# facebookresearch/DRTK

Hardware: AMD Instinct MI355X
Metric: Mpixels/sec fwd+bwd, 100k-tri @ 2048x2048, 1/2/4/8 GPU; HBM BW % (higher is better)
Workload: dtype f32; 1 GPU; 8 views/GPU x 1 GPU, 100k-tri UV-sphere head mesh (F=100352, V=50400), 2048x2048, C=16 attribute channels, transform+rasterize+render+interpolate+mask+edge_grad_estimator+loss fwd+bwd; views_per_gpu=8, triangles=100352, vertices=50400, height=2048, width=2048, channels=16, grad_reset=set_to_none, parallelism=single GPU

## Files before the change

drtk_amd/csrc/edge_grad.hip:

```cpp
#include <cstdlib>

#include "common.hpp"
#include "segscatter.hpp"

namespace drtk_amd {
namespace {

template <typename T>
struct Vec4;
template <>
struct Vec4<float> {
  using type = float4;
};
template <>
struct Vec4<double> {
  using type = double4;
};

template <typename T>
using Quad = T __attribute__((ext_vector_type(4), aligned(sizeof(T))));

template <typename T, int VEC>
struct Row {
  T v[VEC];
  T next;
};

template <typename T, int VEC>
__device__ __forceinline__ Row<T, VEC> load_row(
    const T* __restrict__ plane, int64_t row_off, int x, int W, bool x_ok, int lane) {
  Row<T, VEC> r;
  if (x_ok) {
    if constexpr (VEC == 4) {
      if (x + 4 <= W) {
        const Quad<T> q = *reinterpret_cast<const Quad<T>*>(plane + row_off + x);
        r.v[0] = q.x, r.v[1] = q.y, r.v[2] = q.z, r.v[3] = q.w;
      } else {
#pragma unroll
        for (int j = 0; j < 4; ++j) r.v[j] = x + j < W ? plane[row_off + x + j] : T(0);
      }
    } else {
      r.v[0] = plane[row_off + x];
    }
  } else {
#pragma unroll
    for (int j = 0; j < VEC; ++j) r.v[j] = T(0);
  }
  r.next = __shfl_down(r.v[0], 1);
  return r;
}

#ifndef DRTK_EDGE_SLOTS
#define DRTK_EDGE_SLOTS 64
#endif
#ifndef DRTK_ONEPASS_CAP
#define DRTK_ONEPASS_CAP 512
#endif
#ifndef DRTK_ONEPASS_WAVES
#define DRTK_ONEPASS_WAVES 6
#endif
constexpr int kOnepassCap = DRTK_ONEPASS_CAP;

template <typename T>
struct PairArgs {
  const T* v_pix;
  const int32_t* vi;
  const T* bary_img;
  T* grad_v_pix;
  int64_t V, vi_sN;
  T M;
};

__device__ __forceinline__ int prefix4(int cnt, unsigned long long lt, int& total) {
  const unsigned long long b0 = __ballot(cnt & 1), b1 = __ballot(cnt & 2), b2 = __ballot(cnt & 4);
  total = __popcll(b0) + 2 * __popcll(b1) + 4 * __popcll(b2);
  return __popcll(b0 & lt) + 2 * __popcll(b1 & lt) + 4 * __popcll(b2 & lt);
}

template <typename T, int AXIS, int SLOTS>
__device__ __forceinline__ void scatter_pair_round(
    bool act, int px, int y, T term, const int32_t* __restrict__ idx_n, const T* __restrict__ v_n,
    const int32_t* __restrict__ vi_n, const T* __restrict__ bary_n, int64_t HW, int W, T M, int32_t* keys,
    TableAcc* vals, T* __restrict__ grad_n);

template <typename T, int VEC, int R, int WAVES, bool SCATTER = false>
__global__ __launch_bounds__(WAVES * kWave, SCATTER ? DRTK_ONEPASS_WAVES : 1) void edge_dots_kernel(
    const T* __restrict__ img, const T* __restrict__ grad_output, const int32_t* __restrict__ index_img, int C,
    int H, int W, int strips_x, T* __restrict__ gdx, T* __restrict__ gdy, int strip, T* __restrict__ zero_out,
    int64_t zero_count, PairArgs<T> pairs) {
  static_assert(!SCATTER || (VEC == 4 && 8 * R <= 32 && sizeof(T) == 4), "the pair phase works on four-pixel lanes of float; its flags are one register");
  if (zero_out) {
    const int64_t step = int64_t(gridDim.x) * gridDim.y * blockDim.x;
    for (int64_t i = (int64_t(blockIdx.y) * gridDim.x + blockIdx.x) * blockDim.x + threadIdx.x; i < zero_count; i += step) zero_out[i] = T(0);
  }
  const int64_t HW = int64_t(H) * W;
  const int n = blockIdx.y;
  const int tile = tile_index(strip);
  const int by = tile / strips_x, sx = tile - by * strips_x;
  const int lane = threadIdx.x & (kWave - 1);
  const int y0 = (by * WAVES + threadIdx.x / kWave) * R;
  if (y0 >= H) return;
  const int x = (sx * (kWave - 1) + lane) * VEC;
  const T* img_n = img + int64_t(n) * C * HW;
  const T* go_n = grad_output + int64_t(n) * C * HW;

  bool any_fg = false;
  uint32_t flags = 0;
  {
    const int32_t* idx_n = index_img + int64_t(n) * HW;
    int32_t above[4] = {-1, -1, -1, -1};
#pragma unroll
    for (int r = 0; r <= R; ++r) {
      const int y = y0 + r;
      if (y < H) {
        bool fg = false;
        int32_t first = -1, last = -1;
        int32_t cur[4] = {-1, -1, -1, -1};
        if (x < W) {
          if constexpr (VEC == 4) {
            Quad<int32_t> q;
            if (x + 4 <= W) {
              q = *reinterpret_cast<const Quad<int32_t>*>(idx_n + int64_t(y) * W + x);
            } else {
              const int32_t* rp = idx_n + int64_t(y) * W + x;
              q.x = rp[0], q.y = x + 1 < W ? rp[1] : -1, q.z = x + 2 < W ? rp[2] : -1, q.w = -1;
            }
            fg = (q.x & q.y & q.z & q.w) != -1;
            first = q.x, last = q.w;
            cur[0] = q.x, cur[1] = q.y, cur[2] = q.z, cur[3] = q.w;
          } else {
            first = last = idx_n[int64_t(y) * W + x];
            fg = first != -1;
          }
        }
        int32_t left = __shfl_up(last, 1), right = __shfl_down(first, 1);
        if (lane == 0) left = (x >= 1 && x < W) ? idx_n[int64_t(y) * W + x - 1] : -1;
        if (lane == kWave - 1) right = (x + VEC < W) ? idx_n[int64_t(y) * W + x + VEC] : -1;
        any_fg = any_fg || fg || left != -1 || right != -1;
        if constexpr (SCATTER) {
#pragma unroll
          for (int j = 0; j < 4; ++j) {
            const bool in_x = lane != kWave - 1 && x + j < W - 1;
            if (r > 0 && in_x && above[j] != cur[j]) flags |= 1u << (4 * R + 4 * (r - 1) + j);
            const int32_t nr = j < 3 ? cur[(j + 1) & 3] : right;
            if (r < R && in_x && y < H - 1 && cur[j] != nr) flags |= 1u << (4 * r + j);
            above[j] = cur[j];
          }
        }
      }
    }
  }
  bool load_any = any_fg;
  if constexpr (SCATTER) {
    if (__ballot(flags != 0) == 0) return;
    uint32_t h3 = 0;
#pragma unroll
    for (int r = 0; r < R; ++r) h3 |= flags & (8u << (4 * r));
    const int left_h3 = __shfl_up(static_cast<int>(h3), 1);
    load_any = flags != 0 || (lane > 0 && left_h3 != 0);
  } else {
    if (__ballot(any_fg) == 0) return;
  }
  const bool x_ok = x < W && load_any;

  T ax[R][VEC], ay[R][VEC];
#pragma unroll
  for (int r = 0; r < R; ++r)
#pragma unroll
    for (int j = 0; j < VEC; ++j) ax[r][j] = ay[r][j] = T(0);

  for (int c = 0; c < C; ++c) {
    const T* ip = img_n + int64_t(c) * HW;
    const T* gp = go_n + int64_t(c) * HW;
    Row<T, VEC> ri[R + 1], rg[R + 1];
#pragma unroll
    for (int r = 0; r <= R; ++r) {
      const bool y_ok = (y0 + r) < H;
      ri[r] = load_row<T, VEC>(ip, int64_t(y0 + r) * W, x, W, x_ok && y_ok, lane);
      rg[r] = load_row<T, VEC>(gp, int64_t(y0 + r) * W, x, W, x_ok && y_ok, lane);
    }
#pragma unroll
    for (int r = 0; r < R; ++r) {
#pragma unroll
      for (int j = 0; j < VEC; ++j) {
        const T inext = (j + 1 < VEC) ? ri[r].v[(j + 1) % VEC] : ri[r].next;
        const T gnext = (j + 1 < VEC) ? rg[r].v[(j + 1) % VEC] : rg[r].next;
        ax[r][j] += (inext - ri[r].v[j]) * (T(0.5) * (gnext + rg[r].v[j]));
        ay[r][j] += (ri[r + 1].v[j] - ri[r].v[j]) * (T(0.5) * (rg[r + 1].v[j] + rg[r].v[j]));
      }
    }
  }
  if constexpr (SCATTER) {
    constexpr int kSlots = DRTK_EDGE_SLOTS;
    constexpr int kCap = kOnepassCap;
    __shared__ uint2 s_list[WAVES][kCap];
    __shared__ int32_t t_keys[WAVES][kSlots];
    __shared__ TableAcc t_vals[WAVES][kSlots * 4];
    const int wave = threadIdx.x / kWave;
    const int32_t* idx_n = index_img + int64_t(n) * HW;
    const T* v_n = pairs.v_pix + int64_t(n) * pairs.V * 3;
    const int32_t* vi_n = pairs.vi + int64_t(n) * pairs.vi_sN;
    const T* bary_n = pairs.bary_img + int64_t(n) * 3 * HW;
    T* grad_n = pairs.grad_v_pix + int64_t(n) * pairs.V * 3;
    const int strip_x0 = sx * (kWave - 1) * VEC;

    table_init<kSlots>(t_keys[wave]);
    for (int i = lane; i < kSlots * 4; i += kWave) t_vals[wave][i] = 0;

    const unsigned long long lt = (1ull << lane) - 1ull;
    int grand = 0;
#pragma unroll
    for (int g = 0; g < 2 * R; ++g) {
      int t;
      prefix4(__popc((flags >> (4 * g)) & 15u), lt, t);
      grand += t;
    }
    if (grand <= kCap) {
      int n_h = 0, n_all = 0;
#pragma unroll
      for (int axis = 0; axis < 2; ++axis) {
#pragma unroll
        for (int r = 0; r < R; ++r) {
          const uint32_t f = (flags >> (4 * R * axis + 4 * r)) & 15u;
          int t;
          int pos = n_all + prefix4(__popc(f), lt, t);
          n_all += t;
#pragma unroll
          for (int j = 0; j < 4; ++j) {
            if (f & (1u << j)) s_list[wave][pos++] = make_uint2((r << 8) | (lane * 4 + j), __builtin_bit_cast(uint32_t, axis == 0 ? ax[r][j] : ay[r][j]));
          }
        }
        if (axis == 0) n_h = n_all;
      }
      wave_lds_sync();

      for (int axis = 0; axis < 2; ++axis) {
        const int l_begin = axis == 0 ? 0 : n_h, l_end = axis == 0 ? n_h : n_all;
        for (int t0 = l_begin; t0 < l_end; t0 += kWave) {
          const int t = t0 + lane;
          const bool act = t < l_end;
          int px = 0, y = 0;
          T term = T(0);
          if (act) {
            const uint2 entry = s_list[wave][t];
            y = y0 + static_cast<int>(entry.x >> 8);
            px = strip_x0 + static_cast<int>(entry.x & 255u);
            term = __builtin_bit_cast(float, entry.y);
          }
          if (axis == 0) {
            scatter_pair_round<T, 0, kSlots>(act, px, y, term, idx_n, v_n, vi_n, bary_n, HW, W, pairs.M, t_keys[wave], t_vals[wave], grad_n);
          } else {
            scatter_pair_round<T, 1, kSlots>(act, px, y, term, idx_n, v_n, vi_n, bary_n, HW, W, pairs.M, t_keys[wave], t_vals[wave], grad_n);
          }
        }
      }
    } else {
      static_assert(2 * kCap >= kWave * 8 * R, "the list's storage must hold a strip's terms");
      uint32_t* s_terms = reinterpret_cast<uint32_t*>(s_list[wave]);
#pragma unroll
      for (int q = 0; q < 4 * R; ++q) {
        s_terms[q * kWave + lane] = __builtin_bit_cast(uint32_t, ax[q / 4][q % 4]);
        s_terms[(4 * R + q) * kWave + lane] = __builtin_bit_cast(uint32_t, ay[q / 4][q % 4]);
      }
      wave_lds_sync();
      for (int axis = 0; axis < 2; ++axis) {
#pragma unroll 1
        for (int k = 0; k < 4 * R; ++k) {
          const bool act = (flags >> (4 * R * axis + k)) & 1u;
          if (__ballot(act) == 0) continue;
          const T term = __builtin_bit_cast(float, s_terms[(4 * R * axis + k) * kWave + lane]);
          if (axis == 0) {
            scatter_pair_round<T, 0, kSlots>(act, x + (k & 3), y0 + (k >> 2), term, idx_n, v_n, vi_n, bary_n, HW, W, pairs.M, t_keys[wave], t_vals[wave], grad_n);
          } else {
            scatter_pair_round<T, 1, kSlots>(act, x + (k & 3), y0 + (k >> 2), term, idx_n, v_n, vi_n, bary_n, HW, W, pairs.M, t_keys[wave], t_vals[wave], grad_n);
          }
        }
      }
    }
    wave_lds_sync();
    table_flush<T, TableAcc, kSlots>(t_keys[wave], t_vals[wave], 4, 3, grad_n, 3, 0);
    return;
  }
  if (!x_ok || lane == kWave - 1) return;
  T* ox = gdx + int64_t(n) * HW;
  T* oy = gdy + int64_t(n) * HW;
#pragma unroll
  for (int r = 0; r < R; ++r) {
    const int y = y0 + r;
    if (y >= H) break;
    const int64_t o = int64_t(y) * W + x;
    if constexpr (VEC == 4) {
      if (x + 4 <= W) {
        *reinterpret_cast<Quad<T>*>(ox + o) = Quad<T>{ax[r][0], ax[r][1], ax[r][2], ax[r][3]};
        *reinterpret_cast<Quad<T>*>(oy + o) = Quad<T>{ay[r][0], ay[r][1], ay[r][2], ay[r][3]};
      } else {
#pragma unroll
        for (int j = 0; j < 4; ++j)
          if (x + j < W) ox[o + j] = ax[r][j], oy[o + j] = ay[r][j];
      }
    } else {
      ox[o] = ax[r][0];
      oy[o] = ay[r][0];
    }
  }
}

template <typename T>
struct TriInfo {
  T p0x, p0y, p1x, p1y;
  T v01x, v01y, v02x, v02y, v12x, v12y;
  T den;
  T nx, ny, nz;
  int32_t i0, i1, i2;
};

template <typename T>
__device__ __forceinline__ void load_tri(
    const T* __restrict__ v_n, const int32_t* __restrict__ vi_n, int32_t idx, TriInfo<T>& t) {
  t.i0 = t.i1 = t.i2 = 0;
  if (idx >= 0) {
    const int32_t* f = vi_n + int64_t(idx) * 3;
    t.i0 = f[0], t.i1 = f[1], t.i2 = f[2];
  }
  t.p0x = v_n[3 * (int64_t)t.i0 + 0];
  t.p0y = v_n[3 * (int64_t)t.i0 + 1];
  t.p1x = v_n[3 * (int64_t)t.i1 + 0];
  t.p1y = v_n[3 * (int64_t)t.i1 + 1];
  const T p2x = v_n[3 * (int64_t)t.i2 + 0], p2y = v_n[3 * (int64_t)t.i2 + 1];
  t.v01x = t.p1x - t.p0x;
  t.v01y = t.p1y - t.p0y;
  t.v02x = p2x - t.p0x;
  t.v02y = p2y - t.p0y;
  t.v12x = p2x - t.p1x;
  t.v12y = p2y - t.p1y;
  t.den = t.v01x * t.v02y - t.v01y * t.v02x;
}

template <typename T>
__device__ __forceinline__ bool pix_in_tri(const TriInfo<T>& t, int x, int y) {
  if (t.den != T(0)) {
    const T px = static_cast<T>(x), py = static_cast<T>(y);
    const T vp0x = px - t.p0x, vp0y = py - t.p0y;
    const T vp1x = px - t.p1x, vp1y = py - t.p1y;
    T b0 = vp1y * t.v12x - vp1x * t.v12y;
    T b1 = vp0x * t.v02y - vp0y * t.v02x;
    T b2 = vp0y * t.v01x - vp0x * t.v01y;
    const T s = t.den > T(0) ? T(1) : (t.den < T(0) ? T(-1) : T(0));
    b0 *= s;
    b1 *= s;
    b2 *= s;
    const bool inside = (b0 >= T(0)) && (b1 >= T(0)) && (b2 >= T(0));
    const bool on0 = b0 == T(0), on1 = b1 == T(0), on2 = b2 == T(0);
    const bool pos = t.den > T(0);
    const bool tl0 = pos ? (t.v12y < T(0) || (t.v12y == T(0) && t.v12x > T(0)))
                         : (t.v12y > T(0) || (t.v12y == T(0) && t.v12x < T(0)));
    const bool tl1 = pos ? (t.v02y > T(0) || (t.v02y == T(0) && t.v02x < T(0)))
                         : (t.v02y < T(0) || (t.v02y == T(0) && t.v02x > T(0)));
    const bool tl2 = pos ? (t.v01y < T(0) || (t.v01y == T(0) && t.v01x > T(0)))
                         : (t.v01y > T(0) || (t.v01y == T(0) && t.v01x < T(0)));
    return inside && !((on0 && !tl0) || (on1 && !tl1) || (on2 && !tl2));
  }
  return false;
}

__device__ __forceinline__ float sqrt_t(float x) {
  return __builtin_sqrtf(x);
}
__device__ __forceinline__ double sqrt_t(double x) {
  return __builtin_sqrt(x);
}

template <typename T>
__device__ __forceinline__ void tri_normal(const T* __restrict__ v_n, TriInfo<T>& t) {
  const T* p0 = v_n + 3 * (int64_t)t.i0;
  const T* p1 = v_n + 3 * (int64_t)t.i1;
  const T* p2 = v_n + 3 * (int64_t)t.i2;
  const T ax = p0[0] - p2[0], ay = p0[1] - p2[1], az = p0[2] - p2[2];
  const T bx = p1[0] - p0[0], by = p1[1] - p0[1], bz = p1[2] - p0[2];
  const T cx = ay * bz - az * by;
  const T cy = az * bx - ax * bz;
  const T cz = ax * by - ay * bx;
  const T inv = T(1.0) / sqrt_t(cx * cx + cy * cy + cz * cz);
  t.nx = cx * inv;
  t.ny = cy * inv;
  t.nz = cz * inv;
}

template <typename T>
__device__ __forceinline__ void get_dp_dr(T nvx, T nvy, T nfx, T nfy, T M, T& ox, T& oy) {
  const T inv_v = T(1.0) / sqrt_t(nvx * nvx + nvy * nvy);
  const T nv_x = nvx * inv_v, nv_y = nvy * inv_v;
  const T inv_f = T(1.0) / sqrt_t(nfx * nfx + nfy * nfy);
  const T nf_x = nfx * inv_f, nf_y = nfy * inv_f;
  const T bx = -nf_y, by = nf_x;
  const T d = bx * nv_x + by * nv_y;
  T q;
  if (M > T(0)) {
    const T abs_d = d < T(0) ? -d : d;
    const T abs_bx = bx < T(0) ? -bx : bx;
    const T lim = abs_bx / M;
    const T m = abs_d < lim ? lim : abs_d;
    const T safe_d = (d >= T(0) ? T(1) : T(-1)) * epsclamp(m);
    q = bx / safe_d;
  } else {
    q = bx / epsclamp(d);
  }
  ox = q * nv_x;
  oy = q * nv_y;
}

template <typename T, int AXIS>
__device__ __forceinline__ void eval_pair(
    const T* __restrict__ v_n, TriInfo<T>& tA, TriInfo<T>& tB, int32_t idxA, int32_t idxB, int xa,
    int ya, T grad_dot, T M, T& gA, T& zA, T& gB, T& zB) {
  gA = zA = gB = zB = T(0);
  const bool a_valid = idxA >= 0, b_valid = idxB >= 0;
  const bool both = a_valid && b_valid;
  const int xb = xa + (AXIS == 0 ? 1 : 0), yb = ya + (AXIS == 1 ? 1 : 0);
  const bool a_in_b = both && pix_in_tri(tB, xa, ya);
  const bool b_in_a = both && pix_in_tri(tA, xb, yb);
  const bool a_over_b = a_in_b && !b_in_a;
  const bool b_over_a = b_in_a && !a_in_b;
  const bool inter = a_in_b && b_in_a;
  const bool adjacent = both && !a_in_b && !b_in_a;
  if (!inter) {
    gA = (!a_valid || b_over_a || adjacent) ? T(0) : grad_dot;
    gB = (!b_valid || a_over_b || adjacent) ? T(0) : grad_dot;
  } else {
    tri_normal(v_n, tA);
    tri_normal(v_n, tB);
    const T a_in = AXIS == 0 ? tA.nx : tA.ny;
    const T b_in = AXIS == 0 ? tB.nx : tB.ny;
    T dx, dz;
    get_dp_dr<T>(a_in, tA.nz, b_in, tB.nz, M, dx, dz);
    gA = grad_dot * dx;
    zA = grad_dot * dz;
    get_dp_dr<T>(b_in, tB.nz, a_in, tA.nz, M, dx, dz);
    gB = grad_dot * dx;
    zB = grad_dot * dz;
  }
}

template <typename T>
__device__ __forceinline__ void edge_pixel(
    const T* __restrict__ v_n, const int32_t* __restrict__ vi_n, const T* __restrict__ gdx_n,
    const T* __restrict__ gdy_n, int64_t pix, int x, int y, int W, int32_t ic, int32_t ir, int32_t id,
    int32_t il, int32_t iu, T M, T& ox, T& oy, T& oz, int32_t* centre_vids = nullptr) {
  T cx = T(0), cy = T(0), cz = T(0);
  T rx = T(0), rz = T(0);
  T dy = T(0), dz = T(0);
  TriInfo<T> tc;
  load_tri<T>(v_n, vi_n, ic, tc);
  if (centre_vids) {
    centre_vids[0] = tc.i0, centre_vids[1] = tc.i1, centre_vids[2] = tc.i2;
  }
  T gA, zA, gB, zB;
  if (ic != ir) {
    TriInfo<T> tn;
    load_tri<T>(v_n, vi_n, ir, tn);
    eval_pair<T, 0>(v_n, tc, tn, ic, ir, x, y, gdx_n[pix], M, gA, zA, gB, zB);
    cx += gA;
    cz += zA;
  }
  if (ic != id) {
    TriInfo<T> tn;
    load_tri<T>(v_n, vi_n, id, tn);
    eval_pair<T, 1>(v_n, tc, tn, ic, id, x, y, gdy_n[pix], M, gA, zA, gB, zB);
    cy += gA;
    cz += zA;
  }
  if (il != ic) {
    TriInfo<T> tn;
    load_tri<T>(v_n, vi_n, il, tn);
    eval_pair<T, 0>(v_n, tn, tc, il, ic, x - 1, y, gdx_n[pix - 1], M, gA, zA, gB, zB);
    rx += gB;
    rz += zB;
  }
  if (iu != ic) {
    TriInfo<T> tn;
    load_tri<T>(v_n, vi_n, iu, tn);
    eval_pair<T, 1>(v_n, tn, tc, iu, ic, x, y - 1, gdy_n[pix - W], M, gA, zA, gB, zB);
    dy += gB;
    dz += zB;
  }
  ox = (T(0) + (-rx)) + (-cx);
  oy = (T(0) + (-dy)) + (-cy);
  oz = ((T(0) + (-dz)) + (-rz)) + (-cz);
}

template <typename T>
__global__ __launch_bounds__(kBlock) void edge_gather_kernel(
    const T* __restrict__ v_pix, const int32_t* __restrict__ vi,
    const int32_t* __restrict__ index_img, const T* __restrict__ gdx, const T* __restrict__ gdy,
    int64_t V, int64_t vi_sN, int H, int W, T M, T* __restrict__ out) {
  const int64_t HW = int64_t(H) * W;
  const int n = blockIdx.y;
  const int64_t pix = int64_t(blockIdx.x) * kBlock + threadIdx.x;
  if (pix >= HW) return;
  const int y = static_cast<int>(pix / W);
  const int x = static_cast<int>(pix - int64_t(y) * W);
  const int32_t* idx_n = index_img + int64_t(n) * HW;

  const bool own = (x < W - 1) && (y < H - 1);
  const bool left = (x >= 1) && (y < H - 1);
  const bool up = (y >= 1) && (x < W - 1);
  const int32_t ic = idx_n[pix];
  const int32_t ir = own ? idx_n[pix + 1] : ic;
  const int32_t id = own ? idx_n[pix + W] : ic;
  const int32_t il = left ? idx_n[pix - 1] : ic;
  const int32_t iu = up ? idx_n[pix - W] : ic;
  T ox = T(0), oy = T(0), oz = T(0);
  if (ic != ir || ic != id || ic != il || ic != iu) {
    edge_pixel<T>(
        v_pix + int64_t(n) * V * 3, vi + int64_t(n) * vi_sN, gdx + int64_t(n) * HW, gdy + int64_t(n) * HW, pix,
        x, y, W, ic, ir, id, il, iu, M, ox, oy, oz);
  }
  T* o = out + int64_t(n) * 3 * HW + pix;
  o[0] = ox;
  o[HW] = oy;
  o[2 * HW] = oz;
}

template <typename T>
__global__ __launch_bounds__(kBlock) void edge_gather4_kernel(
    const T* __restrict__ v_pix, const int32_t* __restrict__ vi,
    const int32_t* __restrict__ index_img, const T* __restrict__ gdx, const T* __restrict__ gdy,
    int64_t V, int64_t vi_sN, int H, int W, T M, T* __restrict__ out, int strip) {
  using V4 = typename Vec4<T>::type;
  constexpr int kWaves = kBlock / kWave;
  constexpr int kPix = kWave * 4;
  __shared__ __attribute__((aligned(16))) T s_out[kWaves][3][kPix];
  __shared__ uint16_t s_list[kWaves][kPix];
  __shared__ int32_t s_nb[kWaves][4][kPix];

  const int64_t HW = int64_t(H) * W;
  const int n = blockIdx.y;
  const int wave = threadIdx.x / kWave, lane = threadIdx.x & (kWave - 1);
  const int64_t wave_pix0 = (int64_t(tile_index(strip)) * kWaves + wave) * kPix;
  if (wave_pix0 >= HW) return;
  const int64_t pix0 = wave_pix0 + lane * 4;
  const bool in_range = pix0 < HW;
  const int32_t* idx_n = index_img + int64_t(n) * HW;
  const int y = in_range ? static_cast<int>(pix0 / W) : 0;
  const int x0 = in_range ? static_cast<int>(pix0 - int64_t(y) * W) : 0;

  int32_t c[4] = {-1, -1, -1, -1}, u[4], d[4];
  if (in_range) {
    const int4 q = *reinterpret_cast<const int4*>(idx_n + pix0);
    c[0] = q.x, c[1] = q.y, c[2] = q.z, c[3] = q.w;
  }
#pragma unroll
  for (int j = 0; j < 4; ++j) u[j] = d[j] = c[j];
  if (in_range && y >= 1) {
    const int4 q = *reinterpret_cast<const int4*>(idx_n + pix0 - W);
    u[0] = q.x, u[1] = q.y, u[2] = q.z, u[3] = q.w;
  }
  if (in_range && y < H - 1) {
    const int4 q = *reinterpret_cast<const int4*>(idx_n + pix0 + W);
    d[0] = q.x, d[1] = q.y, d[2] = q.z, d[3] = q.w;
  }
  int32_t lprev = __shfl_up(c[3], 1), rnext = __shfl_down(c[0], 1);
  if (in_range && lane == 0 && x0 >= 1) lprev = idx_n[pix0 - 1];
  if (in_range && lane == kWave - 1 && x0 + 4 < W) rnext = idx_n[pix0 + 4];

  bool e[4];
  int32_t nr[4], nd[4], nl[4], nu[4];
#pragma unroll
  for (int j = 0; j < 4; ++j) {
    const int x = x0 + j;
    const bool own = in_range && (x < W - 1) && (y < H - 1);
    const bool left = in_range && (x >= 1) && (y < H - 1);
    const bool up = in_range && (y >= 1) && (x < W - 1);
    nr[j] = own ? (j < 3 ? c[(j + 1) & 3] : rnext) : c[j];
    nd[j] = own ? d[j] : c[j];
    nl[j] = left ? (j > 0 ? c[(j + 3) & 3] : lprev) : c[j];
    nu[j] = up ? u[j] : c[j];
    e[j] = c[j] != nr[j] || c[j] != nd[j] || c[j] != nl[j] || c[j] != nu[j];
  }

  const V4 zero4 = V4{T(0), T(0), T(0), T(0)};
#pragma unroll
  for (int k = 0; k < 3; ++k) *reinterpret_cast<V4*>(&s_out[wave][k][lane * 4]) = zero4;
  *reinterpret_cast<int4*>(&s_nb[wave][0][lane * 4]) = make_int4(nr[0], nr[1], nr[2], nr[3]);
  *reinterpret_cast<int4*>(&s_nb[wave][1][lane * 4]) = make_int4(nd[0], nd[1], nd[2], nd[3]);
  *reinterpret_cast<int4*>(&s_nb[wave][2][lane * 4]) = make_int4(nl[0], nl[1], nl[2], nl[3]);
  *reinterpret_cast<int4*>(&s_nb[wave][3][lane * 4]) = make_int4(nu[0], nu[1], nu[2], nu[3]);
  const unsigned long long lt = (1ull << lane) - 1ull;
  int total = 0;
#pragma unroll
  for (int j = 0; j < 4; ++j) {
    const unsigned long long m = __ballot(e[j]);
    if (e[j]) s_list[wave][total + __popcll(m & lt)] = static_cast<uint16_t>(lane * 4 + j);
    total += __popcll(m);
  }
  wave_lds_sync();

  const T* v_n = v_pix + int64_t(n) * V * 3;
  const int32_t* vi_n = vi + int64_t(n) * vi_sN;
  const T* gdx_n = gdx + int64_t(n) * HW;
  const T* gdy_n = gdy + int64_t(n) * HW;
  for (int t0 = 0; t0 < total; t0 += kWave) {
    const int t = t0 + lane;
    if (t < total) {
      const int local = s_list[wave][t];
      const int64_t pix = wave_pix0 + local;
      const int py = static_cast<int>(pix / W);
      const int px = static_cast<int>(pix - int64_t(py) * W);
      const int32_t ic = idx_n[pix];
      T ox, oy, oz;
      edge_pixel<T>(
          v_n, vi_n, gdx_n, gdy_n, pix, px, py, W, ic, s_nb[wave][0][local], s_nb[wave][1][local],
          s_nb[wave][2][local], s_nb[wave][3][local], M, ox, oy, oz);
      s_out[wave][0][local] = ox;
      s_out[wave][1][local] = oy;
      s_out[wave][2][local] = oz;
    }
  }
  wave_lds_sync();
  if (in_range) {
    T* o = out + int64_t(n) * 3 * HW + pix0;
#pragma unroll
    for (int k = 0; k < 3; ++k) *reinterpret_cast<V4*>(o + int64_t(k) * HW) = *reinterpret_cast<const V4*>(&s_out[wave][k][lane * 4]);
  }
}

template <typename T, int AXIS, int SLOTS>
__device__ __forceinline__ void scatter_pair_round(
    bool act, int px, int y, T term, const int32_t* __restrict__ idx_n, const T* __restrict__ v_n,
    const int32_t* __restrict__ vi_n, const T* __restrict__ bary_n, int64_t HW, int W, T M, int32_t* keys,
    TableAcc* vals, T* __restrict__ grad_n) {
  int32_t ia = -1, ib = -1;
  T ga = T(0), za = T(0), gb = T(0), zb = T(0);
  T Ba[3] = {T(0), T(0), T(0)}, Bb[3] = {T(0), T(0), T(0)};
  int32_t va[3] = {0, 0, 0}, vb[3] = {0, 0, 0};
  if (act) {
    const int64_t pa = int64_t(y) * W + px;
    const int64_t pb = AXIS == 0 ? pa + 1 : pa + W;
    ia = idx_n[pa];
    ib = idx_n[pb];
    TriInfo<T> ta, tb;
    load_tri<T>(v_n, vi_n, ia, ta);
    load_tri<T>(v_n, vi_n, ib, tb);
    T gA, zA, gB, zB;
    eval_pair<T, AXIS>(v_n, ta, tb, ia, ib, px, y, term, M, gA, zA, gB, zB);
    ga = -gA, za = -zA, gb = -gB, zb = -zB;
    va[0] = ta.i0, va[1] = ta.i1, va[2] = ta.i2;
    vb[0] = tb.i0, vb[1] = tb.i1, vb[2] = tb.i2;
    if (ia >= 0) Ba[0] = bary_n[pa], Ba[1] = bary_n[HW + pa], Ba[2] = bary_n[2 * HW + pa];
    if (ib >= 0) Bb[0] = bary_n[pb], Bb[1] = bary_n[HW + pb], Bb[2] = bary_n[2 * HW + pb];
  }
  const bool a_on = ia >= 0 && (ga != T(0) || za != T(0));
  const bool b_on = ib >= 0 && (gb != T(0) || zb != T(0));
  T g[12];
#pragma unroll
  for (int k = 0; k < 3; ++k) {
    g[2 * k + 0] = a_on ? ga * Ba[k] : T(0);
    g[2 * k + 1] = a_on ? za * Ba[k] : T(0);
    g[6 + 2 * k + 0] = b_on ? gb * Bb[k] : T(0);
    g[6 + 2 * k + 1] = b_on ? zb * Bb[k] : T(0);
  }
  const int32_t key_a = a_on ? ia : -1, key_b = b_on ? ib : -1;
  int dist;
  bool tail;
  const int32_t left_a = __shfl_up(key_a, 1), left_b = __shfl_up(key_b, 1);
  run_rows16_heads(key_a != left_a || key_b != left_b, dist, tail);
  if (__ballot(a_on || b_on) != 0) {
    run_sums_rows16<T, 12>(g, dist);
    constexpr int c_off = AXIS == 0 ? 0 : 1, c_step = AXIS == 0 ? 2 : 1;
    if (tail && a_on) table_add<T, 3, 2, SLOTS>(keys, vals, 4, va, g, grad_n, 3, c_off, c_step);
    if (tail && b_on) table_add<T, 3, 2, SLOTS>(keys, vals, 4, vb, g + 6, grad_n, 3, c_off, c_step);
  }
}

#ifndef DRTK_PAIR_ROWS
#define DRTK_PAIR_ROWS 2
#endif
constexpr int kPairRows = DRTK_PAIR_ROWS;
template <typename T>
__global__ __launch_bounds__(kBlock, sizeof(T) == 4 ? 4 : 2) void edge_scatter_pairs_kernel(
    const T* __restrict__ v_pix, const int32_t* __restrict__ vi, const int32_t* __restrict__ index_img,
    const T* __restrict__ bary_img, const T* __restrict__ gdx, const T* __restrict__ gdy, int64_t V, int64_t vi_sN,
    int H, int W, int strips_x, T M, T* __restrict__ grad_v_pix, int strip) {
  constexpr int kWaves = kBlock / kWave;
  constexpr int kRows = kPairRows;
  constexpr int kCap = kWave * 4 * 2 * 2;
  __shared__ uint16_t s_list[kWaves][kCap];
  constexpr int kSlots = DRTK_EDGE_SLOTS;
  __shared__ int32_t t_keys[kWaves][kSlots];
  __shared__ TableAcc t_vals[kWaves][kSlots * 4];

  const int64_t HW = int64_t(H) * W;
  const int n = blockIdx.y;
  const int wave = threadIdx.x / kWave, lane = threadIdx.x & (kWave - 1);
  const int wg = tile_index(strip) * kWaves + wave;
  const int ry = wg / strips_x, sx = wg - ry * strips_x;
  const int y_base = ry * kRows;
  if (y_base >= H) return;
  const int x0 = (sx * kWave + lane) * 4;
  const bool in_x = x0 < W;
  const int32_t* idx_n = index_img + int64_t(n) * HW;
  const T* v_n = v_pix + int64_t(n) * V * 3;
  const int32_t* vi_n = vi + int64_t(n) * vi_sN;
  const T* gdx_n = gdx + int64_t(n) * HW;
  const T* gdy_n = gdy + int64_t(n) * HW;
  const T* bary_n = bary_img + int64_t(n) * 3 * HW;
  T* grad_n = grad_v_pix + int64_t(n) * V * 3;

  table_init<kSlots>(t_keys[wave]);
  for (int i = lane; i < kSlots * 4; i += kWave) t_vals[wave][i] = 0;

  int32_t row[kRows + 1][4];
#pragma unroll
  for (int r = 0; r <= kRows; ++r) {
    const int y = y_base + r;
    if (in_x && y < H) {
      const int32_t* rp = idx_n + int64_t(y) * W + x0;
      if (x0 + 4 <= W) {
        const Quad<int32_t> q = *reinterpret_cast<const Quad<int32_t>*>(rp);
        row[r][0] = q.x, row[r][1] = q.y, row[r][2] = q.z, row[r][3] = q.w;
      } else {
#pragma unroll
        for (int j = 0; j < 4; ++j) row[r][j] = x0 + j < W ? rp[j] : -1;
      }
    } else {
#pragma unroll
      for (int j = 0; j < 4; ++j) row[r][j] = -1;
    }
  }
  uint32_t hf[kRows], vf[kRows];
#pragma unroll
  for (int r = 0; r < kRows; ++r) {
    const int y = y_base + r;
    int32_t rnext = __shfl_down(row[r][0], 1);
    if (in_x && y < H && lane == kWave - 1 && x0 + 4 < W) rnext = idx_n[int64_t(y) * W + x0 + 4];
    hf[r] = vf[r] = 0;
#pragma unroll
    for (int j = 0; j < 4; ++j) {
      const bool own = in_x && (x0 + j < W - 1) && (y < H - 1);
      const int32_t nr = j < 3 ? row[r][(j + 1) & 3] : rnext;
      if (own && row[r][j] != nr) hf[r] |= 1u << j;
      if (own && row[r][j] != row[r + 1][j]) vf[r] |= 1u << j;
    }
  }
  const unsigned long long lt = (1ull << lane) - 1ull;

  int grand = 0;
#pragma unroll
  for (int r = 0; r < kRows; ++r) {
    int t;
    prefix4(__popc(hf[r]), lt, t);
    grand += t;
    prefix4(__popc(vf[r]), lt, t);
    grand += t;
  }
  const int rows_per_group = grand <= kCap ? kRows : (kRows < 2 ? kRows : 2);
  for (int r0 = 0; r0 < kRows; r0 += rows_per_group) {
    int n_h = 0, n_all = 0;
    wave_lds_sync();
#pragma unroll
    for (int axis = 0; axis < 2; ++axis) {
#pragma unroll
      for (int r = 0; r < kRows; ++r) {
        if (r < r0 || r >= r0 + rows_per_group) continue;
        const uint32_t f = axis == 0 ? hf[r] : vf[r];
        int t;
        int pos = n_all + prefix4(__popc(f), lt, t);
        n_all += t;
#pragma unroll
        for (int j = 0; j < 4; ++j) {
          if (f & (1u << j)) s_list[wave][pos++] = static_cast<uint16_t>((r << 8) | (lane * 4 + j));
        }
      }
      if (axis == 0) n_h = n_all;
    }
    wave_lds_sync();

    for (int axis = 0; axis < 2; ++axis) {
      const int l_begin = axis == 0 ? 0 : n_h, l_end = axis == 0 ? n_h : n_all;
      for (int t0 = l_begin; t0 < l_end; t0 += kWave) {
        const int t = t0 + lane;
        const bool act = t < l_end;
        int px = 0, y = 0;
        T term = T(0);
        if (act) {
          const int entry = s_list[wave][t];
          y = y_base + (entry >> 8);
          px = sx * (kWave * 4) + (entry & 255);
          term = (axis == 0 ? gdx_n : gdy_n)[int64_t(y) * W + px];
        }
        if (axis == 0) {
          scatter_pair_round<T, 0, kSlots>(act, px, y, term, idx_n, v_n, vi_n, bary_n, HW, W, M, t_keys[wave], t_vals[wave], grad_n);
        } else {
          scatter_pair_round<T, 1, kSlots>(act, px, y, term, idx_n, v_n, vi_n, bary_n, HW, W, M, t_keys[wave], t_vals[wave], grad_n);
        }
      }
    }
  }
  wave_lds_sync();
  table_flush<T, TableAcc, kSlots>(t_keys[wave], t_vals[wave], 4, 3, grad_n, 3, 0);
}

#ifndef DRTK_DOTS_ROWS
#define DRTK_DOTS_ROWS 2
#endif
#ifndef DRTK_DOTS_WAVES
#define DRTK_DOTS_WAVES 4
#endif
constexpr int kStripRows = DRTK_DOTS_ROWS;
constexpr int kDotsWaves = DRTK_DOTS_WAVES;

template <typename T>
int edge_grad_backward_impl(
    const T* v_pix, const T* img, const int32_t* index_img, const int32_t* vi, const T* grad_output,
    int64_t N, int64_t V, int64_t C, int64_t vi_sN, int64_t H, int64_t W, double max_dp_dr, T* out,
    void* workspace, hipStream_t stream) {
  const int64_t HW = H * W;
  if (N * HW == 0) return DRTK_OK;
  T* gdx = static_cast<T*>(workspace);
  T* gdy = gdx + N * HW;
  const bool vec = (W % 4 == 0) && (reinterpret_cast<uintptr_t>(img) % (4 * sizeof(T)) == 0) &&
      (reinterpret_cast<uintptr_t>(grad_output) % (4 * sizeof(T)) == 0) &&
      (reinterpret_cast<uintptr_t>(workspace) % (4 * sizeof(T)) == 0) &&
      (reinterpret_cast<uintptr_t>(index_img) % 16 == 0);
  const int px_per_wave = (kWave - 1) * 4;
  const int strips_x = static_cast<int>(ceil_div(W, px_per_wave));
  const int bands_y = static_cast<int>(ceil_div(H, kStripRows * kDotsWaves));
  const dim3 gridA(static_cast<unsigned>(int64_t(strips_x) * bands_y), static_cast<unsigned>(N));
  DRTK_LAUNCH((edge_dots_kernel<T, 4, kStripRows, kDotsWaves>), gridA, dim3(kDotsWaves * kWave), 0, stream, img, grad_output, index_img, (int)C, (int)H, (int)W, strips_x, gdx, gdy, xcd_strip(int64_t(strips_x) * (16 / (kStripRows * kDotsWaves))), static_cast<T*>(nullptr), int64_t(0), PairArgs<T>{});
  DRTK_RETURN_IF_LAUNCH_FAILED();
  const bool vec_out = vec && (reinterpret_cast<uintptr_t>(index_img) % 16 == 0) &&
      (reinterpret_cast<uintptr_t>(out) % (4 * sizeof(T)) == 0);
  if (vec_out) {
    const dim3 gridB(static_cast<unsigned>(ceil_div(HW, kBlock * 4)), static_cast<unsigned>(N));
    DRTK_LAUNCH((edge_gather4_kernel<T>), gridB, dim3(kBlock), 0, stream, v_pix, vi, index_img, gdx, gdy, V, vi_sN, (int)H, (int)W, static_cast<T>(max_dp_dr), out, xcd_strip(ceil_div(16 * W, kBlock * 4)));
  } else {
    const dim3 gridB(static_cast<unsigned>(ceil_div(HW, kBlock)), static_cast<unsigned>(N));
    DRTK_LAUNCH((edge_gather_kernel<T>), gridB, dim3(kBlock), 0, stream, v_pix, vi, index_img, gdx, gdy, V, vi_sN, (int)H, (int)W, static_cast<T>(max_dp_dr), out);
  }
  DRTK_RETURN_IF_LAUNCH_FAILED();
  return DRTK_OK;
}

template <typename T>
int launch_edge_dots(const T* img, const T* grad_output, const int32_t* index_img, int64_t N, int64_t C, int64_t H, int64_t W, T* gdx, T* gdy, hipStream_t stream, T* zero_out, int64_t zero_count) {
  const int px_per_wave = (kWave - 1) * 4;
  const int strips_x = static_cast<int>(ceil_div(W, px_per_wave));
  const int bands_y = static_cast<int>(ceil_div(H, kStripRows * kDotsWaves));
  const dim3 gridA(static_cast<unsigned>(int64_t(strips_x) * bands_y), static_cast<unsigned>(N));
  DRTK_LAUNCH((edge_dots_kernel<T, 4, kStripRows, kDotsWaves>), gridA, dim3(kDotsWaves * kWave), 0, stream, img, grad_output, index_img, (int)C, (int)H, (int)W, strips_x, gdx, gdy, xcd_strip(int64_t(strips_x) * (16 / (kStripRows * kDotsWaves))), zero_out, zero_count, PairArgs<T>{});
  DRTK_RETURN_IF_LAUNCH_FAILED();
  return DRTK_OK;
}

inline bool aligned_to(const void* p, size_t a) {
  return reinterpret_cast<uintptr_t>(p) % a == 0;
}

#ifndef DRTK_EDGE_ONEPASS
#define DRTK_EDGE_ONEPASS 1
#endif
#ifndef DRTK_EDGE_ONEPASS_MIN_PX
#define DRTK_EDGE_ONEPASS_MIN_PX (int64_t(1) << 20)
#endif
inline bool edge_onepass_wanted(int64_t pixels) {
  const char* e = std::getenv("DRTK_AMD_EDGE_ONEPASS");
  if (e && e[0] && !e[1] && (e[0] == '0' || e[0] == '1')) return e[0] == '1';
  return pixels >= DRTK_EDGE_ONEPASS_MIN_PX;
}

template <typename T>
int edge_grad_backward_fused_impl(
    drtk_dtype_t dtype, const T* v_pix, const T* img, const int32_t* index_img, const int32_t* vi,
    const T* bary_img, const T* grad_output, int64_t N, int64_t V, int64_t C, int64_t F, int64_t vi_sN,
    int64_t H, int64_t W, double max_dp_dr, T* grad_v_pix, void* workspace, size_t workspace_bytes,
    hipStream_t stream) {
  const int64_t HW = H * W;
  if (N * HW == 0) {
    if (N * V > 0 && fill_bytes_async(grad_v_pix, 0, sizeof(T) * N * V * 3, stream) != DRTK_OK) return DRTK_ERR_LAUNCH;
    return DRTK_OK;
  }
#if DRTK_EDGE_ONEPASS
  if constexpr (std::is_same<T, float>::value) {
    if (edge_onepass_wanted(N * HW)) {
      if (N * V > 0 && fill_bytes_async(grad_v_pix, 0, sizeof(T) * N * V * 3, stream) != DRTK_OK) return DRTK_ERR_LAUNCH;
      const int strips_x = static_cast<int>(ceil_div(W, (kWave - 1) * 4));
      const int bands_y = static_cast<int>(ceil_div(H, kStripRows * kDotsWaves));
      const dim3 grid(static_cast<unsigned>(int64_t(strips_x) * bands_y), static_cast<unsigned>(N));
      const PairArgs<T> pairs{v_pix, vi, bary_img, grad_v_pix, V, vi_sN, static_cast<T>(max_dp_dr)};
      DRTK_LAUNCH((edge_dots_kernel<T, 4, kStripRows, kDotsWaves, true>), grid, dim3(kDotsWaves * kWave), 0, stream, img, grad_output, index_img, (int)C, (int)H, (int)W, strips_x, static_cast<T*>(nullptr), static_cast<T*>(nullptr), xcd_strip(int64_t(strips_x) * (16 / (kStripRows * kDotsWaves))), static_cast<T*>(nullptr), int64_t(0), pairs);
      DRTK_RETURN_IF_LAUNCH_FAILED();
      return DRTK_OK;
    }
  }
#endif
  T* gdx = static_cast<T*>(workspace);
  T* gdy = gdx + N * HW;
  const int st = launch_edge_dots<T>(img, grad_output, index_img, N, C, H, W, gdx, gdy, stream, grad_v_pix, N * V * 3);
  if (st != DRTK_OK) return st;
  const int strips_x = static_cast<int>(ceil_div(W, kWave * 4));
  const int64_t waves = int64_t(strips_x) * ceil_div(H, kPairRows);
  const dim3 grid(static_cast<unsigned>(ceil_div(waves, kBlock / kWave)), static_cast<unsigned>(N));
  const int strip = xcd_strip(ceil_div(int64_t(strips_x) * (16 / kPairRows), kBlock / kWave));
  DRTK_LAUNCH((edge_scatter_pairs_kernel<T>), grid, dim3(kBlock), 0, stream, v_pix, vi, index_img, bary_img, gdx, gdy, V, vi_sN, (int)H, (int)W, strips_x, static_cast<T>(max_dp_dr), grad_v_pix, strip);
  DRTK_RETURN_IF_LAUNCH_FAILED();
  return DRTK_OK;
}

}
}

using namespace drtk_amd;

extern "C" int drtk_amd_edge_grad_backward_workspace_bytes(
    drtk_dtype_t dtype, int64_t N, int64_t H, int64_t W, size_t* bytes) {
  if (!bytes || N < 0 || H < 0 || W < 0 || (dtype != DRTK_F32 && dtype != DRTK_F64)) return DRTK_ERR_INVALID_ARGUMENT;
  const size_t es = dtype == DRTK_F32 ? 4 : 8;
  const size_t b = size_t(2) * N * H * W * es;
  *bytes = b > 0 ? b : 16;
  return DRTK_OK;
}

extern "C" int drtk_amd_edge_grad_backward(
    drtk_dtype_t dtype, const void* v_pix, const void* img, const int32_t* index_img,
    const int32_t* vi, const void* grad_output, int64_t N, int64_t V, int64_t C, int64_t F,
    int64_t vi_sN, int64_t H, int64_t W, double max_dp_dr, void* grad_v_pix_img, void* workspace,
    size_t workspace_bytes, drtk_stream_t stream) {
  if (N < 0 || V < 0 || C < 0 || F < 0 || H < 0 || W < 0 ||
      (vi_sN != 0 && vi_sN != F * 3) || H * W >= (int64_t(1) << 31) || (dtype != DRTK_F32 && dtype != DRTK_F64))
    return DRTK_ERR_INVALID_ARGUMENT;
  if (reinterpret_cast<uintptr_t>(workspace) % 16 != 0) return DRTK_ERR_INVALID_ARGUMENT;
  size_t need = 0;
  if (drtk_amd_edge_grad_backward_workspace_bytes(dtype, N, H, W, &need) != DRTK_OK) return DRTK_ERR_INVALID_ARGUMENT;
  if (N * H * W > 0) {
    if (!index_img || !grad_v_pix_img || !workspace) return DRTK_ERR_INVALID_ARGUMENT;
    if ((N * V > 0 && !v_pix) || (F > 0 && !vi)) return DRTK_ERR_INVALID_ARGUMENT;
    if (C > 0 && (!img || !grad_output)) return DRTK_ERR_INVALID_ARGUMENT;
    if (workspace_bytes < need) return DRTK_ERR_WORKSPACE_TOO_SMALL;
  }
  {
    const size_t es = dtype_size(dtype);
    DRTK_FOR_VIEW_SLICES(N, n0, n, drtk_amd_edge_grad_backward(
        dtype, advance(v_pix, n0 * V * 3, es), advance(img, n0 * C * H * W, es), advance_typed(index_img, n0 * H * W),
        advance_typed(vi, n0 * vi_sN), advance(grad_output, n0 * C * H * W, es), n, V, C, F, vi_sN, H, W, max_dp_dr,
        advance(grad_v_pix_img, n0 * 3 * H * W, es), workspace, workspace_bytes, stream))
  }
  hipStream_t s = static_cast<hipStream_t>(stream);
  switch (dtype) {
    case DRTK_F32:
      return edge_grad_backward_impl<float>(static_cast<const float*>(v_pix), static_cast<const float*>(img), index_img, vi, static_cast<const float*>(grad_output), N, V, C, vi_sN, H, W, max_dp_dr, static_cast<float*>(grad_v_pix_img), workspace, s);
    case DRTK_F64:
      return edge_grad_backward_impl<double>(static_cast<const double*>(v_pix), static_cast<const double*>(img), index_img, vi, static_cast<const double*>(grad_output), N, V, C, vi_sN, H, W, max_dp_dr, static_cast<double*>(grad_v_pix_img), workspace, s);
    default:
      return DRTK_ERR_INVALID_ARGUMENT;
  }
}

extern "C" int drtk_amd_edge_grad_backward_fused_workspace_bytes(
    drtk_dtype_t dtype, int64_t N, int64_t H, int64_t W, size_t* bytes) {
  if (!bytes || N < 0 || H < 0 || W < 0 || (dtype != DRTK_F32 && dtype != DRTK_F64)) return DRTK_ERR_INVALID_ARGUMENT;
  const size_t es = dtype == DRTK_F32 ? 4 : 8;
  const size_t b = size_t(2) * N * H * W * es;
  *bytes = b > 0 ? b : 16;
  return DRTK_OK;
}

extern "C" int drtk_amd_edge_grad_backward_fused(
    drtk_dtype_t dtype, const void* v_pix, const void* img, const int32_t* index_img,
    const int32_t* vi, const void* bary_img, const void* grad_output, int64_t N, int64_t V, int64_t C,
    int64_t F, int64_t vi_sN, int64_t H, int64_t W, double max_dp_dr, void* grad_v_pix,
    void* workspace, size_t workspace_bytes, drtk_stream_t stream) {
  if (N < 0 || V < 0 || C < 0 || F < 0 || H < 0 || W < 0 ||
      (vi_sN != 0 && vi_sN != F * 3) || H * W >= (int64_t(1) << 31) || (dtype != DRTK_F32 && dtype != DRTK_F64))
    return DRTK_ERR_INVALID_ARGUMENT;
  if (reinterpret_cast<uintptr_t>(workspace) % 16 != 0) return DRTK_ERR_INVALID_ARGUMENT;
  size_t need = 0;
  if (drtk_amd_edge_grad_backward_fused_workspace_bytes(dtype, N, H, W, &need) != DRTK_OK) return DRTK_ERR_INVALID_ARGUMENT;
  if (N * V > 0 && !grad_v_pix) return DRTK_ERR_INVALID_ARGUMENT;
  if (N * H * W > 0) {
    if (!index_img || !bary_img || !workspace) return DRTK_ERR_INVALID_ARGUMENT;
    if ((N * V > 0 && !v_pix) || (F > 0 && !vi)) return DRTK_ERR_INVALID_ARGUMENT;
    if (C > 0 && (!img || !grad_output)) return DRTK_ERR_INVALID_ARGUMENT;
    if (workspace_bytes < need) return DRTK_ERR_WORKSPACE_TOO_SMALL;
  }
  {
    const size_t es = dtype_size(dtype);
    DRTK_FOR_VIEW_SLICES(N, n0, n, drtk_amd_edge_grad_backward_fused(
        dtype, advance(v_pix, n0 * V * 3, es), advance(img, n0 * C * H * W, es), advance_typed(index_img, n0 * H * W),
        advance_typed(vi, n0 * vi_sN), advance(bary_img, n0 * 3 * H * W, es), advance(grad_output, n0 * C * H * W, es), n, V, C, F,
        vi_sN, H, W, max_dp_dr, advance(grad_v_pix, n0 * V * 3, es), workspace, workspace_bytes, stream))
  }
  hipStream_t s = static_cast<hipStream_t>(stream);
  switch (dtype) {
    case DRTK_F32:
      return edge_grad_backward_fused_impl<float>(dtype, static_cast<const float*>(v_pix), static_cast<const float*>(img), index_img, vi, static_cast<const float*>(bary_img), static_cast<const float*>(grad_output), N, V, C, F, vi_sN, H, W, max_dp_dr, static_cast<float*>(grad_v_pix), workspace, workspace_bytes, s);
    case DRTK_F64:
      return edge_grad_backward_fused_impl<double>(dtype, static_cast<const double*>(v_pix), static_cast<const double*>(img), index_img, vi, static_cast<const double*>(bary_img), static_cast<const double*>(grad_output), N, V, C, F, vi_sN, H, W, max_dp_dr, static_cast<double*>(grad_v_pix), workspace, workspace_bytes, s);
    default:
      return DRTK_ERR_INVALID_ARGUMENT;
  }
}
```

Before: 6637 Mpix/s.

## Prune edge pairs whose triangles never cover each other's pixel before loading channels

Adds a pre-pass in the fused edge-dots/scatter kernel. It lists each flagged boundary pair and loads both triangles, then keeps only pairs where one pixel lies inside the other pixel's triangle. Strips with no surviving pairs exit before the C-channel image and gradient loads, and fewer pairs reach the scatter phase. The cost is extra triangle loads, point-in-triangle tests, LDS atomics and syncs. The shared buffers move to kernel scope so the pre-pass can reuse them.

```diff
diff --git a/drtk_amd/csrc/edge_grad.hip b/drtk_amd/csrc/edge_grad.hip
--- a/drtk_amd/csrc/edge_grad.hip
+++ b/drtk_amd/csrc/edge_grad.hip
@@ -60,6 +60,9 @@
 #define DRTK_ONEPASS_WAVES 6
 #endif
 constexpr int kOnepassCap = DRTK_ONEPASS_CAP;
+#ifndef DRTK_EDGE_PRUNE
+#define DRTK_EDGE_PRUNE 1
+#endif
 
 template <typename T>
 struct PairArgs {
@@ -83,12 +86,22 @@
     const int32_t* __restrict__ vi_n, const T* __restrict__ bary_n, int64_t HW, int W, T M, int32_t* keys,
     TableAcc* vals, T* __restrict__ grad_n);
 
+template <typename T, int R>
+__device__ __forceinline__ uint32_t needed_pair_flags(
+    uint32_t flags, int lane, int strip_x0, int y0, const int32_t* __restrict__ idx_n, const T* __restrict__ v_n,
+    const int32_t* __restrict__ vi_n, int W, uint32_t* list, uint32_t* mask);
+
 template <typename T, int VEC, int R, int WAVES, bool SCATTER = false>
 __global__ __launch_bounds__(WAVES * kWave, SCATTER ? DRTK_ONEPASS_WAVES : 1) void edge_dots_kernel(
     const T* __restrict__ img, const T* __restrict__ grad_output, const int32_t* __restrict__ index_img, int C,
     int H, int W, int strips_x, T* __restrict__ gdx, T* __restrict__ gdy, int strip, T* __restrict__ zero_out,
     int64_t zero_count, PairArgs<T> pairs) {
   static_assert(!SCATTER || (VEC == 4 && 8 * R <= 32 && sizeof(T) == 4), "the pair phase works on four-pixel lanes of float; its flags are one register");
+  constexpr int kSlots = DRTK_EDGE_SLOTS;
+  constexpr int kCap = kOnepassCap;
+  __shared__ uint2 s_list[SCATTER ? WAVES : 1][SCATTER ? kCap : 1];
+  __shared__ int32_t t_keys[SCATTER ? WAVES : 1][SCATTER ? kSlots : 1];
+  __shared__ TableAcc t_vals[SCATTER ? WAVES : 1][SCATTER ? kSlots * 4 : 1];
   if (zero_out) {
     const int64_t step = int64_t(gridDim.x) * gridDim.y * blockDim.x;
     for (int64_t i = (int64_t(blockIdx.y) * gridDim.x + blockIdx.x) * blockDim.x + threadIdx.x; i < zero_count; i += step) zero_out[i] = T(0);
@@ -153,6 +166,16 @@
   bool load_any = any_fg;
   if constexpr (SCATTER) {
     if (__ballot(flags != 0) == 0) return;
+#if DRTK_EDGE_PRUNE
+    {
+      static_assert(2 * kCap >= (kWave - 1) * 8 * R && kSlots >= kWave, "the list's storage must hold a strip's pair positions, the keys' one word per lane");
+      const int wave = __builtin_amdgcn_readfirstlane(threadIdx.x / kWave);
+      flags = needed_pair_flags<T, R>(
+          flags, lane, sx * (kWave - 1) * VEC, y0, index_img + int64_t(n) * HW, pairs.v_pix + int64_t(n) * pairs.V * 3,
+          pairs.vi + int64_t(n) * pairs.vi_sN, W, reinterpret_cast<uint32_t*>(s_list[wave]), reinterpret_cast<uint32_t*>(t_keys[wave]));
+      if (__ballot(flags != 0) == 0) return;
+    }
+#endif
     uint32_t h3 = 0;
 #pragma unroll
     for (int r = 0; r < R; ++r) h3 |= flags & (8u << (4 * r));
@@ -191,12 +214,7 @@
     }
   }
   if constexpr (SCATTER) {
-    constexpr int kSlots = DRTK_EDGE_SLOTS;
-    constexpr int kCap = kOnepassCap;
-    __shared__ uint2 s_list[WAVES][kCap];
-    __shared__ int32_t t_keys[WAVES][kSlots];
-    __shared__ TableAcc t_vals[WAVES][kSlots * 4];
-    const int wave = threadIdx.x / kWave;
+    const int wave = __builtin_amdgcn_readfirstlane(threadIdx.x / kWave);
     const int32_t* idx_n = index_img + int64_t(n) * HW;
     const T* v_n = pairs.v_pix + int64_t(n) * pairs.V * 3;
     const int32_t* vi_n = pairs.vi + int64_t(n) * pairs.vi_sN;
@@ -672,6 +690,52 @@
   }
 }
 
+template <typename T, int R>
+__device__ __forceinline__ uint32_t needed_pair_flags(
+    uint32_t flags, int lane, int strip_x0, int y0, const int32_t* __restrict__ idx_n, const T* __restrict__ v_n,
+    const int32_t* __restrict__ vi_n, int W, uint32_t* list, uint32_t* mask) {
+  const unsigned long long lt = (1ull << lane) - 1ull;
+  mask[lane] = 0;
+  int n_all = 0;
+#pragma unroll
+  for (int g = 0; g < 2 * R; ++g) {
+    const uint32_t f = (flags >> (4 * g)) & 15u;
+    int t;
+    int pos = n_all + prefix4(__popc(f), lt, t);
+    n_all += t;
+#pragma unroll
+    for (int j = 0; j < 4; ++j) {
+      if (f & (1u << j)) list[pos++] = static_cast<uint32_t>((lane << 5) | (4 * g + j));
+    }
+  }
+  wave_lds_sync();
+  for (int t0 = 0; t0 < n_all; t0 += kWave) {
+    const int t = t0 + lane;
+    if (t < n_all) {
+      const uint32_t entry = list[t];
+      const int bit = static_cast<int>(entry & 31u), owner = static_cast<int>(entry >> 5);
+      const bool vertical = bit >= 4 * R;
+      const int k = vertical ? bit - 4 * R : bit;
+      const int xa = strip_x0 + owner * 4 + (k & 3), ya = y0 + (k >> 2);
+      const int xb = vertical ? xa : xa + 1, yb = vertical ? ya + 1 : ya;
+      const int64_t pa = int64_t(ya) * W + xa;
+      const int32_t ia = idx_n[pa], ib = idx_n[vertical ? pa + W : pa + 1];
+      bool need = true;
+      if (ia >= 0 && ib >= 0) {
+        TriInfo<T> ta, tb;
+        load_tri<T>(v_n, vi_n, ia, ta);
+        load_tri<T>(v_n, vi_n, ib, tb);
+        const bool a_in_b = pix_in_tri(tb, xa, ya);
+        const bool b_in_a = pix_in_tri(ta, xb, yb);
+        need = a_in_b || b_in_a;
+      }
+      if (need) atomicOr(&mask[owner], 1u << bit);
+    }
+  }
+  wave_lds_sync();
+  return mask[lane];
+}
+
 #ifndef DRTK_PAIR_ROWS
 #define DRTK_PAIR_ROWS 2
 #endif
```

Measured after the change: 7162 Mpix/s, median of 6. 7.9% higher.
